# klasmodin/quflow

Measured on AMD Instinct MI355X. Metric: isospectral timesteps/sec at N=1024 (1 GPU) + ensemble steps/sec at 1/2/4/8 GPUs, higher is better.
Workload: dtype f64

## Files before the change

quflow_amd/csrc/api_context.hip:

```cpp
#include <cmath>
#include <cstdarg>
#include <cstdio>
#include <cstdlib>
#include <cstring>
#include <limits>
#include <chrono>

#include "qf_api.h"

static thread_local char g_err[512] = "";

void qf_set_error(const char *fmt, ...)
{
    va_list ap;
    va_start(ap, fmt);
    vsnprintf(g_err, sizeof(g_err), fmt, ap);
    va_end(ap);
}

extern "C" {

int qf_version(void) { return QF_VERSION; }

int qf_device_info(int device, char *buf, int n)
// ... 92 lines not shown
        if (g[0] == 'i' && strstr(g, "x6")) ctx->oz_digits = 6;
        if (g[0] == 'i' && strstr(g, "x65")) ctx->oz_digits2 = 5;
        if (g[0] == 'i' && strchr(g, 'h')) ctx->gemm_i8_hybrid = true;
        if (g[0] == 'i' && strchr(g, 'f') && !ctx->gemm_i8_hybrid) ctx->gemm_i8_first = true;
        if (g[0] == 'a') {
            ctx->gemm_i8_allowed = true;
            ctx->oz_digits = 6;
            ctx->oz_digits2 = 5;
            ctx->gemm_i8_min_n = 1024;
        }
    }
    if (const char *g = getenv("QUFLOW_HIP_GEMM2")) ctx->gemm_tri_allowed = !(g[0] == 'f');
    if (const char *g = getenv("QUFLOW_HIP_FUSED")) ctx->fused_allowed = !(g[0] == '0');
    if (const char *g = getenv("QUFLOW_HIP_I8_MIN_N")) ctx->gemm_i8_min_n = atoi(g);
    if (const char *g = getenv("QUFLOW_HIP_TRI_MIN_N")) ctx->gemm_tri_min_n = atoi(g);
    if (const char *g = getenv("QUFLOW_HIP_DEFER")) ctx->defer_allowed = !(g[0] == '0');
    if (getenv("QUFLOW_HIP_DEBUG"))
        if (const char *g = getenv("QUFLOW_HIP_DEBUG_DROP_FLAG")) ctx->debug_drop = atoi(g);
    if (const char *g = getenv("QUFLOW_HIP_FACTOR_CACHE_MB")) ctx->factor_budget_bytes = (size_t)(atoi(g) > 0 ? atoi(g) : 1) << 20;
    const size_t NN = (size_t)N * N;
    const size_t mbytes = NN * sizeof(cplx);
    int rc = QF_OK;
    auto fail = [&](int code) {
        qf_ctx_destroy(ctx);
        return code;
    };
#define QF_CREATE_HIP(call)                                                                   \
    do {                                                                                      \
        hipError_t _e = (call);                                                               \
        if (_e != hipSuccess) {                                                               \
// ... 288 lines not shown
```

quflow_amd/csrc/api_isomp.hip:

```cpp
#include <cmath>
#include <cstdarg>
#include <cstdio>
#include <cstdlib>
#include <cstring>
#include <limits>
#include <chrono>
#include <type_traits>
#include <utility>

#include "qf_api.h"

namespace {

#ifndef QF_RUN_AHEAD
#define QF_RUN_AHEAD 3
#endif

template <class S> constexpr bool is_c64 = std::is_same<S, qf_c64>::value;

template <class S> S *ws(qf_ctx *ctx)
{
    if constexpr (is_c64<S>) return ctx->c64;
    else return ctx;
}
// ... 61 lines not shown
        int so = 2, sd = 1;
        {
            const int cus = ctx->num_cus > 0 ? ctx->num_cus : 256;
            if (nt * (nt - 1) + 2 * nt <= cus) sd = 2;
            else if (nt * (nt - 1) + nt > cus) so = 1;
        }
        ctx->tri32_split = so;
        ctx->tri32_split_diag = sd;
    }
    return QF_OK;
}

int select_second_product(qf_ctx *ctx)
{
    ctx->gemm_tri = false;
    ctx->gemm_tri32 = false;
    ctx->gemm_i8 = false;
    const bool want_tri = ctx->gemm_tri_allowed && ctx->sk_partial && ctx->N >= ctx->gemm_tri_min_n;
    const size_t nt32 = (size_t)(ctx->N + 31) / 32;
    const bool tri32_fits = nt32 * (nt32 + 1) / 2 * 4 * 32 * 32 * sizeof(cplx) <= (size_t)0x7fffffff;
    const bool want_tri32 = ctx->gemm_tri_allowed && !want_tri && ctx->N >= 64 && tri32_fits;
    const bool want_i8 = ctx->gemm_i8_allowed && ctx->N % 64 == 0 && ctx->N >= ctx->gemm_i8_min_n && ctx->N <= 4096;
    if (!want_tri && !want_i8 && !want_tri32) return QF_OK;
    QF_TRY(check_skew(ctx, ctx));
    const bool skew = ctx->w_skew_known;
    ctx->gemm_tri = want_tri && skew;
    ctx->gemm_i8 = want_i8 && skew;
    ctx->gemm_tri32 = want_tri32 && skew && (!ctx->gemm_i8 || ctx->gemm_i8_first);
    if (ctx->gemm_tri32) QF_TRY(tri32_alloc(ctx));
    return QF_OK;
}

int select_second_product_c64(qf_ctx *ctx)
{
    qf_c64 *f = ctx->c64;
    f->tri = false;
    if (f->tri_allowed && ctx->gemm_tri_allowed && (qf_c64_tile(ctx) == 32 || ctx->N % 64 == 0) && ctx->N >= 64) {
        QF_TRY(check_skew(ctx, f));
        if (f->w_skew_known) {
            QF_TRY(qf_c64_tri_alloc(ctx));
            f->tri = true;
// ... 723 lines not shown
        QF_TRY(qf_launch_mirror_lower(ctx, f->dW[1]));
        QF_TRY(qf_launch_sum_rowpart(ctx, f->rowpart, (N + qf_c64_tile(ctx) - 1) / qf_c64_tile(ctx), ctx->rowsum));
    } else {
        QF_TRY(qf_launch_cgemm(ctx, f->PW, f->Phalf, nullptr, &ep));
        QF_TRY(qf_launch_sum_rowpart(ctx, f->rowpart, f->rowpart_tiles, ctx->rowsum));
    }
    QF_HIP(hipMemcpyAsync(dW_new_host, f->dW[1], bytes, hipMemcpyDeviceToHost, ctx->stream));
    QF_HIP(hipMemcpyAsync(Whalf_new_host, f->Whalf, bytes, hipMemcpyDeviceToHost, ctx->stream));
    QF_HIP(hipMemcpyAsync(rowsum_host, ctx->rowsum, (size_t)N * sizeof(double), hipMemcpyDeviceToHost, ctx->stream));
    QF_HIP(hipStreamSynchronize(ctx->stream));
    return QF_OK;
}

}

int qf_rowpart_slots(const qf_ctx *ctx) { return ctx->gemm_tri ? ctx->N / 64 : ctx->gemm_tri32 ? (ctx->N + 31) / 32 : ctx->rowpart_tiles; }

int qf_enqueue_diagnostics(qf_ctx *ctx)
{
    QF_TRY(qf_launch_solve(ctx, ctx->poisson, ctx->W, ctx->stage, 1.0, 1));
    QF_TRY(qf_launch_inner2(ctx, ctx->W, ctx->stage, ctx->scalars + 2));
    QF_HIP(hipMemcpyAsync(ctx->host_scalars, ctx->scalars + 2, 2 * sizeof(double), hipMemcpyDeviceToHost, ctx->stream));
    return QF_OK;
}

int qf_isomp_multi(qf_ctx **ctxs, int k, double dt, int steps, double tol, int minit, int maxit, qf_isomp_stats *stats_out)
{
    return isomp_multi<qf_ctx>(ctxs, k, dt, steps, tol, minit, maxit, stats_out);
}

int qf_c64_isomp_multi(qf_ctx **ctxs, int k, double dt, int steps, double tol, int minit, int maxit, qf_isomp_stats *stats_out)
// ... 30 lines not shown
    return QF_OK;
}


int qf_fixedpoint_products(qf_ctx *ctx, const void *Phalf_host, const void *Whalf_host, const void *W_host,
                           const void *dW_old_host, int variant, void *dW_new_host, void *Whalf_new_host,
                           double *rowsum_host)
{
    QF_TRY(check_ctx(ctx));
    if (!Phalf_host || !Whalf_host || !W_host || !dW_old_host || !dW_new_host || !Whalf_new_host || !rowsum_host) {
        qf_set_error("qf_fixedpoint_products: null buffer");
        return QF_ERR_INVALID;
    }
    const int variant_arg = variant;
    variant &= 15;
    if (variant == 1 && !ctx->sk_partial) {
        qf_set_error("qf_fixedpoint_products: the upper-triangle product needs N %% 64 == 0 (N=%d)", ctx->N);
        return QF_ERR_INVALID;
    }
    if (variant == 2) {
        if (ctx->N < 64) {
            qf_set_error("qf_fixedpoint_products: the 32x32 upper-triangle product needs N >= 64 (N=%d)", ctx->N);
            return QF_ERR_INVALID;
        }
        QF_TRY(tri32_alloc(ctx));
    }
    const int N = ctx->N;
    const size_t bytes = (size_t)N * N * sizeof(cplx);
    QF_HIP(hipMemcpyAsync(ctx->Phalf, Phalf_host, bytes, hipMemcpyHostToDevice, ctx->stream));
    QF_HIP(hipMemcpyAsync(ctx->Whalf, Whalf_host, bytes, hipMemcpyHostToDevice, ctx->stream));
    QF_HIP(hipMemcpyAsync(ctx->stage, W_host, bytes, hipMemcpyHostToDevice, ctx->stream));
    QF_HIP(hipMemcpyAsync(ctx->dW[0], dW_old_host, bytes, hipMemcpyHostToDevice, ctx->stream));
    QF_TRY(qf_launch_zgemm(ctx, ctx->Phalf, ctx->Whalf, ctx->PW, nullptr));
    qf_epilogue ep = epilogue_of(ctx, false);
    ep.W = ctx->stage;
    const bool saved = ctx->gemm_tri, saved32 = ctx->gemm_tri32;
    const int s_min = ctx->sk_min_units, s_epi = ctx->sk_epi_units, s_so = ctx->tri32_split, s_sd = ctx->tri32_split_diag;
    ctx->gemm_tri = (variant == 1);
    ctx->gemm_tri32 = (variant == 2);
    if (variant == 1) {
        if ((variant_arg >> 8) & 0xff) ctx->sk_min_units = (variant_arg >> 8) & 0xff;
        if ((variant_arg >> 16) & 0xff) ctx->sk_epi_units = ((variant_arg >> 16) & 0xff) - 64;
    } else if (variant == 2) {
        const int so = (variant_arg >> 8) & 15, sd = (variant_arg >> 12) & 15;
        if (so == 1 || so == 2 || so == 4) ctx->tri32_split = so;
        if (sd == 1 || sd == 2 || sd == 4) ctx->tri32_split_diag = sd;
    }
    int rc = qf_launch_zgemm(ctx, ctx->PW, ctx->Phalf, nullptr, &ep);
    ctx->gemm_tri = saved;
    ctx->gemm_tri32 = saved32;
    ctx->sk_min_units = s_min;
    ctx->sk_epi_units = s_epi;
    ctx->tri32_split = s_so;
    ctx->tri32_split_diag = s_sd;
    QF_TRY(rc);
    QF_TRY(qf_launch_sum_rowpart(ctx, ctx->rowpart, variant == 1 ? ctx->N / 64 : variant == 2 ? (ctx->N + 31) / 32 : ctx->rowpart_tiles, ctx->rowsum));
    QF_HIP(hipMemcpyAsync(dW_new_host, ctx->dW[1], bytes, hipMemcpyDeviceToHost, ctx->stream));
    QF_HIP(hipMemcpyAsync(Whalf_new_host, ctx->Whalf, bytes, hipMemcpyDeviceToHost, ctx->stream));
    QF_HIP(hipMemcpyAsync(rowsum_host, ctx->rowsum, (size_t)N * sizeof(double), hipMemcpyDeviceToHost, ctx->stream));
    QF_HIP(hipStreamSynchronize(ctx->stream));
    return QF_OK;
}


int qf_oz_alloc(qf_ctx *ctx)
{
    for (int q = 0; q < 4; ++q) {
        if (!ctx->oz_planes[q]) QF_HIP(hipMalloc((void **)&ctx->oz_planes[q], qf_oz_operand_bytes(ctx->N, ctx->oz_digits)));
        if (!ctx->oz_scale[q])
            QF_HIP(hipMalloc((void **)&ctx->oz_scale[q], qf_oz_record_bytes(ctx->N, ctx->oz_digits)));
    }
// ... 39 lines not shown
```

quflow_amd/csrc/api_steppers.hip:

```cpp
#include <cmath>
#include <cstdarg>
#include <cstdio>
#include <cstdlib>
#include <cstring>
#include <limits>
#include <chrono>

#include "qf_api.h"

extern "C" {

int qf_erk(qf_ctx *ctx, int method, double dt, int steps, int skewh)
{
    QF_TRY(check_ctx(ctx));
    if (method < QF_ERK_EULER || method > QF_ERK_RK4) {
        qf_set_error("qf_erk: unknown method %d", method);
        return QF_ERR_INVALID;
    }
    if (steps < 0) {
        qf_set_error("qf_erk: steps must be >= 0");
        return QF_ERR_INVALID;
    }
    const double inv_hb = 1.0 / qf_hbar(ctx->N);
    ctx->w_skew_known = false;
// ... 396 lines not shown
        QF_HIP(hipMemcpyAsync(S[j].X, (const char *)states_host + (size_t)j * mbytes, mbytes, hipMemcpyHostToDevice, ctx->stream));
        QF_HIP(hipMemsetAsync(S[j].dX[0], 0, mbytes, ctx->stream));
        QF_HIP(hipMemcpyAsync(S[j].Xhalf, S[j].X, mbytes, hipMemcpyDeviceToDevice, ctx->stream));
    }
    cplx *Bhalf = magnetic ? ctx->multi[5 * k] : nullptr;
    cplx *BT = magnetic ? ctx->multi[5 * k + 1] : nullptr;
    cplx *BTP = magnetic ? ctx->multi[5 * k + 2] : nullptr;

    bool tri = ctx->gemm_tri_allowed && ctx->sk_partial && N >= ctx->gemm_tri_min_n;
    for (int j = 0; j < k && tri; ++j) {
        QF_TRY(qf_launch_skew_defect(ctx, S[j].X, ctx->scalars + 4));
        QF_HIP(hipMemcpyAsync(ctx->host_scalars, ctx->scalars + 4, 2 * sizeof(double), hipMemcpyDeviceToHost, ctx->stream));
        QF_HIP(hipStreamSynchronize(ctx->stream));
        tri = (ctx->host_scalars[0] == 0.0);
    }
    const bool tri_saved = ctx->gemm_tri, tri32_saved = ctx->gemm_tri32;
    ctx->gemm_tri = tri;
    ctx->gemm_tri32 = false;
    auto restore = [&](int rc) { ctx->gemm_tri = tri_saved; ctx->gemm_tri32 = tri32_saved; return rc; };
#define QF_TRY_R(call)                  \
    do {                                \
        int _r = (call);                \
        if (_r != QF_OK) return restore(_r); \
    } while (0)

    if (tol < 0) {
        double nrm = 0.0;
        QF_TRY_R(qf_launch_norm_inf(ctx, S[0].X, ctx->scalars));
        QF_TRY_R(read_scalar(ctx, ctx->scalars, &nrm));
        tol = (std::sqrt(std::numeric_limits<double>::epsilon()) * dt / hb) * nrm;
    }

    long long total_iterations = 0, number_of_maxit = 0;
    double resnorm = 0.0;
// ... 56 lines not shown
                }
            }
        }
        if (!broke) number_of_maxit += 1;
        for (int j = 0; j < k; ++j)
            QF_TRY_R(qf_launch_update(ctx, S[j].PXc, S[j].X, S[j].dX[S[j].cur], S[j].dX[S[j].cur], S[j].Xhalf, nullptr,
                                      reinitialize));
        if (magnetic)
            QF_TRY_R(qf_launch_magnetic_update(ctx, BT, S[0].X, reinitialize ? nullptr : S[0].dX[S[0].cur], S[0].Xhalf));
    }
    for (int j = 0; j < k; ++j)
        QF_HIP(hipMemcpyAsync((char *)states_host + (size_t)j * mbytes, S[j].X, mbytes, hipMemcpyDeviceToHost, ctx->stream));
    QF_HIP(hipStreamSynchronize(ctx->stream));
#undef QF_TRY_R
    ctx->gemm_tri = tri_saved;
    ctx->gemm_tri32 = tri32_saved;
    if (stats_out) {
        stats_out->total_iterations = total_iterations;
        stats_out->number_of_maxit = number_of_maxit;
        stats_out->tol_used = tol;
        stats_out->last_resnorm = resnorm;
    }
    return QF_OK;
}


}
```

quflow_amd/csrc/qf_api.h:

```cpp
#pragma once

#include "qf_internal.h"

#include <sched.h>

namespace {
int drain_events(qf_ctx *ctx);

struct prof_scope {
    qf_ctx *ctx;
    qf_event_pair ev;
    bool active;
    prof_scope(qf_ctx *c, int id) : ctx(c), active(((c->profile_mask >> id) & 1) != 0)
    {
        ctx->plan_role = id;
        if (!active) return;
        if ((ctx->prof_seen[id]++ % ctx->profile_stride) != 0) {
            active = false;
            return;
        }
        if (ctx->events_free.empty()) {
            if (hipEventCreate(&ev.start) != hipSuccess || hipEventCreate(&ev.stop) != hipSuccess) {
                active = false;
                return;
// ... 48 lines not shown
}

int read_scalar(qf_ctx *ctx, const double *dev, double *out)
{
    QF_HIP(hipMemcpyAsync(ctx->host_scalars, dev, sizeof(double), hipMemcpyDeviceToHost, ctx->stream));
    QF_HIP(hipStreamSynchronize(ctx->stream));
    *out = ctx->host_scalars[0];
    return QF_OK;
}

}

extern "C" {
int qf_need_c64(qf_ctx *ctx);
int qf_oz_alloc(qf_ctx *ctx);
int qf_rowpart_slots(const qf_ctx *ctx);
int qf_enqueue_diagnostics(qf_ctx *ctx);
}
```

quflow_amd/csrc/qf_internal.h:

```cpp
#pragma once

#include <hip/hip_runtime.h>

#include <atomic>
#include <cstdarg>
#include <cstdio>
#include <map>
#include <mutex>
#include <string>
#include <vector>

#include "../../include/quflow_hip.h"

typedef double2 cplx;

hipError_t qf_guard_malloc(void **p, size_t bytes);
hipError_t qf_guard_free(void *p);
#define hipMalloc(p, n) qf_guard_malloc((void **)(p), (n))
#define hipFree(p) qf_guard_free((void *)(p))

void qf_set_error(const char *fmt, ...);
struct qf_ctx;
inline void qf_plan_note(qf_ctx *ctx, unsigned long long key, const char *fmt, ...) __attribute__((format(printf, 3, 4)));

// ... 262 lines not shown
    qf_sht sht;
    qf_eigh_ws eigh;

    double *rowpart = nullptr;
    int rowpart_tiles = 0;
    double *rowsum = nullptr;
    double *scalars = nullptr;
    double *host_scalars = nullptr;
    qf_dev_state *state = nullptr;
    qf_host_record *host_rec = nullptr;
    bool diag_at_exit = false, diag_valid = false;
    unsigned *ticket = nullptr;
    int pred_iters = 3;
    bool gemm_tri_allowed = true;
    bool gemm_tri = false;
    int gemm_tri_min_n = 960;
    bool gemm_tri32 = false;
    int tri32_split = 2, tri32_split_diag = 1;
    cplx *t32_partial = nullptr;
    unsigned *t32_arrive = nullptr;
    bool defer_allowed = true;
    bool defer = false;
    int num_cus = 0;
    cplx *sk_partial = nullptr;
    unsigned *sk_flags = nullptr;
    int sk_slots = 0;
    unsigned sk_epoch = 0;
    int sk_epi_units = 0;
    int sk_epi_units_fused = 2;
    int sk_min_units = 8;
// ... 174 lines not shown
```

quflow_amd/csrc/zgemm.hip:

```cpp
#include "qf_internal.h"
#include "qf_step_end.h"

#include <cstring>

typedef double v4d __attribute__((ext_vector_type(4)));

#ifdef QF_STAMP
__device__ unsigned long long *qf_stamp_buf = nullptr;
#define QF_STAMP_SLOTS 80
#ifdef QF_STAMP_LIGHT
#define QF_STAMP_AT(slot_)
#define QF_STAMP_PH(kt_, ph_)
__device__ unsigned long long *qf_phase_buf = nullptr;
#else
#define QF_STAMP_AT(slot_)                                                              \
    if (qf_stamp_buf && lane == 0 && (slot_) < QF_STAMP_SLOTS)                          \
        qf_stamp_buf[((size_t)blockIdx.x * (T / 64) + wave) * QF_STAMP_SLOTS + (slot_)] = __builtin_amdgcn_s_memtime();
__device__ unsigned long long *qf_phase_buf = nullptr;
#define QF_STAMP_PH(kt_, ph_)                                                           \
    if (qf_phase_buf && tid == 0 && (kt_) >= 20 && (kt_) < 28)                          \
        qf_phase_buf[((size_t)blockIdx.x * 8 + ((kt_) - 20)) * 5 + (ph_)] = __builtin_amdgcn_s_memtime();
#endif
__device__ unsigned long long *qf_tri_buf = nullptr;
#define QF_TRI_STAMP(seg_, k_)                                                          \
// ... 973 lines not shown
        t = n_t;
        k0 = n_k0;
        KT = n_KT;
        tm = n_tm;
        tn = n_tn;
        asm volatile("s_waitcnt lgkmcnt(0)\n\ts_barrier" ::: "memory");
    }
    if (run_finale)
        qf_fused_step_end(N, nt, ep.rowpart, sk.ticket, sk.state_rw, sk.rec, guard.iter, tid, reinterpret_cast<double *>(smem_raw));
#undef QF_TRI_NEXT
#undef QF_TRI_KOF
#undef QF_TRI_HAS_PIECE
#undef QF_TRI_START_LOADS
}

template <bool EXACT>
__global__ __launch_bounds__(256) void k_zgemm_tri32(int N, int nt, const cplx *__restrict__ A, const cplx *__restrict__ B,
                                                      qf_epilogue ep, qf_guard guard, qf_tri32 sx)
{
    if (!qf_guard_iter(guard)) return;
    constexpr int BM = 32, BN = 32, WM = 2, WN = 2;
    constexpr bool EPI = true, FAST = false;
    using SM = tile_smem<BM, BN, false>;
    constexpr int T = WM * WN * 64;
    constexpr int WTM = BM / WM, WTN = BN / WN;
    constexpr int MT = WTM / 16, NT = WTN / 16;
    static_assert(MT == 1 && NT == 1, "one MFMA tile per wave");
    constexpr int A_STRIDE = SM::A_STRIDE, B_STRIDE = SM::B_STRIDE;
    constexpr int A_PER = (BM * BK) / T, B_PER = (BN * BK) / T;
    constexpr int A_ROWS_PER = T / BK, B_ROWS_PER = T / BN;
// ... 363 lines not shown
}

int qf_gemm_tiles_n(int N)
{
    gemm_cfg c = pick_gemm(N);
    return (N + c.BN - 1) / c.BN;
}

int qf_launch_zgemm_tri(qf_ctx *ctx, const cplx *A, const cplx *B, const qf_epilogue *ep, qf_guard guard)
{
    const int N = ctx->N;
    if (!ep || N % 64 != 0 || !ctx->sk_partial || ctx->num_cus < 1) {
        qf_set_error("qf_launch_zgemm_tri: not available for this context (N=%d)", N);
        return QF_ERR_STATE;
    }
    static qf_smem_attr attr;
    QF_TRY(qf_smem_attr_set(attr, (const void *)k_zgemm_tri, ctx->device, TRI_SMEM_BYTES));
    const int nt = N / 64;
    int E = ep->fused ? ctx->sk_epi_units_fused : ctx->sk_epi_units;
    if (E < -8) E = -8;
    const long long units = (long long)nt * (nt + 1) / 2 * (N / BK + E);
    if (units > 0x7fffffffLL) {
        qf_set_error("qf_launch_zgemm_tri: N=%d is too large for the stream-K partition", N);
        return QF_ERR_INVALID;
    }
    long long grid_ll = units / (ctx->sk_min_units > 0 ? ctx->sk_min_units : 1);
    if (grid_ll > ctx->num_cus) grid_ll = ctx->num_cus;
    if (grid_ll < 1) grid_ll = 1;
    const int grid = (int)grid_ll;
    qf_streamk sk;
    const int slots = ctx->sk_slots > 0 ? ctx->sk_slots : ctx->num_cus;
    sk.slots = slots;
    sk.partial = ctx->sk_partial;
    sk.flags = ctx->sk_flags;
    sk.epoch = ++ctx->sk_epoch;
    sk.fault = &ctx->host_rec->fault;
    sk.ticket = ctx->sk_flags + slots;
    sk.n_tiles = nt * (nt + 1) / 2;
    sk.state_rw = ctx->state;
    sk.rec = ctx->host_rec;
    if (ctx->debug_drop == 1 || (ctx->debug_drop == 2 && ep->fused)) {
        sk.debug_drop = ctx->debug_drop;
        sk.spin_limit = 1u << 14;
        ctx->debug_drop = 0;
    }
    qf_plan_note(ctx, 0x2000000ull | (unsigned long long)(grid << 8 | (E & 0x3f) << 1 | (ep->fused ? 1 : 0)),
                 "{\"kernel\": \"k_zgemm_tri\", \"arithmetic\": \"fp64 3M, v_mfma_f64_16x16x4_f64\", \"tile\": [64, 64], \"tiles\": %d, "
                 "\"tile_share\": %.6f, \"workgroups\": %d, \"threads\": 256, \"partition\": \"stream-K over (tile, K-tile) units, "
                 "contiguous ranges, epilogue weight E = %d K-tiles\", \"step_end\": \"%s\"}",
                 sk.n_tiles, (double)sk.n_tiles / ((double)nt * nt), grid, E, ep->fused ? "fused (last finisher decides)" : "two-kernel");
    hipLaunchKernelGGL(k_zgemm_tri, dim3(grid), dim3(256), TRI_SMEM_BYTES, ctx->stream, N, nt, (int)units, E, A, B, *ep, guard, sk);
    QF_HIP(hipGetLastError());
    return QF_OK;
}

int qf_launch_zgemm_tri32(qf_ctx *ctx, const cplx *A, const cplx *B, const qf_epilogue *ep, qf_guard guard)
{
    const int N = ctx->N;
    if (!ep || N < 64 || !ctx->t32_partial || !ctx->t32_arrive) {
        qf_set_error("qf_launch_zgemm_tri32: not available for this context (N=%d)", N);
        return QF_ERR_STATE;
    }
    const int nt = (N + 31) / 32;
    qf_tri32 sx;
    sx.partial = ctx->t32_partial;
    sx.arrive = ctx->t32_arrive;
// ... 36 lines not shown
```

Before: 2699.

## Add half-tile stream-K units for triangular ZGEMM when tiles underfill CUs

Adds a k_zgemm_tri_half kernel that splits each 64x64 upper-triangle tile into two 64x32 column halves, doubling the number of stream-K work units. It is selected automatically when the triangular tile count is below the CU count but at least half of it, and N is at most 1024. The goal is better CU load balance and less idle hardware in the second fixed-point product. In exchange, tiles are smaller with lower data reuse, the epilogue and mirroring logic gets more complex, and there are more rowpart slots to sum.

New measurement: 2692. Within noise of the previous version (-0.3%).

```diff
diff --git a/quflow_amd/csrc/api_context.hip b/quflow_amd/csrc/api_context.hip
--- a/quflow_amd/csrc/api_context.hip
+++ b/quflow_amd/csrc/api_context.hip
@@ -130,6 +130,7 @@
     if (const char *g = getenv("QUFLOW_HIP_FUSED")) ctx->fused_allowed = !(g[0] == '0');
     if (const char *g = getenv("QUFLOW_HIP_I8_MIN_N")) ctx->gemm_i8_min_n = atoi(g);
     if (const char *g = getenv("QUFLOW_HIP_TRI_MIN_N")) ctx->gemm_tri_min_n = atoi(g);
+    if (const char *g = getenv("QUFLOW_HIP_TRI_UNIT")) ctx->tri_unit_mode = (g[0] == 't') ? 1 : (g[0] == 'h') ? 2 : 0;
     if (const char *g = getenv("QUFLOW_HIP_DEFER")) ctx->defer_allowed = !(g[0] == '0');
     if (getenv("QUFLOW_HIP_DEBUG"))
         if (const char *g = getenv("QUFLOW_HIP_DEBUG_DROP_FLAG")) ctx->debug_drop = atoi(g);
diff --git a/quflow_amd/csrc/api_isomp.hip b/quflow_amd/csrc/api_isomp.hip
--- a/quflow_amd/csrc/api_isomp.hip
+++ b/quflow_amd/csrc/api_isomp.hip
@@ -99,6 +99,7 @@
 int select_second_product(qf_ctx *ctx)
 {
     ctx->gemm_tri = false;
+    ctx->gemm_tri_half = false;
     ctx->gemm_tri32 = false;
     ctx->gemm_i8 = false;
     const bool want_tri = ctx->gemm_tri_allowed && ctx->sk_partial && ctx->N >= ctx->gemm_tri_min_n;
@@ -110,6 +111,7 @@
     QF_TRY(check_skew(ctx, ctx));
     const bool skew = ctx->w_skew_known;
     ctx->gemm_tri = want_tri && skew;
+    ctx->gemm_tri_half = ctx->gemm_tri && qf_tri_half_units(ctx);
     ctx->gemm_i8 = want_i8 && skew;
     ctx->gemm_tri32 = want_tri32 && skew && (!ctx->gemm_i8 || ctx->gemm_i8_first);
     if (ctx->gemm_tri32) QF_TRY(tri32_alloc(ctx));
@@ -863,7 +865,15 @@
 
 }
 
-int qf_rowpart_slots(const qf_ctx *ctx) { return ctx->gemm_tri ? ctx->N / 64 : ctx->gemm_tri32 ? (ctx->N + 31) / 32 : ctx->rowpart_tiles; }
+bool qf_tri_half_units(const qf_ctx *ctx)
+{
+    if (ctx->N % 64 != 0 || !ctx->sk_partial || ctx->tri_unit_mode == 1) return false;
+    if (ctx->tri_unit_mode == 2) return true;
+    const int nt = ctx->N / 64, n_tiles = nt * (nt + 1) / 2;
+    return n_tiles < ctx->num_cus && ctx->num_cus <= 2 * n_tiles && ctx->N <= ctx->tri_half_max_n;
+}
+
+int qf_rowpart_slots(const qf_ctx *ctx) { return ctx->gemm_tri ? (ctx->gemm_tri_half ? ctx->N / 32 : ctx->N / 64) : ctx->gemm_tri32 ? (ctx->N + 31) / 32 : ctx->rowpart_tiles; }
 
 int qf_enqueue_diagnostics(qf_ctx *ctx)
 {
@@ -924,7 +934,7 @@
     }
     const int variant_arg = variant;
     variant &= 15;
-    if (variant == 1 && !ctx->sk_partial) {
+    if ((variant == 1 || variant == 3) && !ctx->sk_partial) {
         qf_set_error("qf_fixedpoint_products: the upper-triangle product needs N %% 64 == 0 (N=%d)", ctx->N);
         return QF_ERR_INVALID;
     }
@@ -944,11 +954,12 @@
     QF_TRY(qf_launch_zgemm(ctx, ctx->Phalf, ctx->Whalf, ctx->PW, nullptr));
     qf_epilogue ep = epilogue_of(ctx, false);
     ep.W = ctx->stage;
-    const bool saved = ctx->gemm_tri, saved32 = ctx->gemm_tri32;
+    const bool saved = ctx->gemm_tri, saved32 = ctx->gemm_tri32, saved_half = ctx->gemm_tri_half;
     const int s_min = ctx->sk_min_units, s_epi = ctx->sk_epi_units, s_so = ctx->tri32_split, s_sd = ctx->tri32_split_diag;
-    ctx->gemm_tri = (variant == 1);
+    ctx->gemm_tri = (variant == 1 || variant == 3);
+    ctx->gemm_tri_half = (variant == 3);
     ctx->gemm_tri32 = (variant == 2);
-    if (variant == 1) {
+    if (variant == 1 || variant == 3) {
         if ((variant_arg >> 8) & 0xff) ctx->sk_min_units = (variant_arg >> 8) & 0xff;
         if ((variant_arg >> 16) & 0xff) ctx->sk_epi_units = ((variant_arg >> 16) & 0xff) - 64;
     } else if (variant == 2) {
@@ -958,13 +969,14 @@
     }
     int rc = qf_launch_zgemm(ctx, ctx->PW, ctx->Phalf, nullptr, &ep);
     ctx->gemm_tri = saved;
+    ctx->gemm_tri_half = saved_half;
     ctx->gemm_tri32 = saved32;
     ctx->sk_min_units = s_min;
     ctx->sk_epi_units = s_epi;
     ctx->tri32_split = s_so;
     ctx->tri32_split_diag = s_sd;
     QF_TRY(rc);
-    QF_TRY(qf_launch_sum_rowpart(ctx, ctx->rowpart, variant == 1 ? ctx->N / 64 : variant == 2 ? (ctx->N + 31) / 32 : ctx->rowpart_tiles, ctx->rowsum));
+    QF_TRY(qf_launch_sum_rowpart(ctx, ctx->rowpart, variant == 1 ? ctx->N / 64 : (variant == 2 || variant == 3) ? (ctx->N + 31) / 32 : ctx->rowpart_tiles, ctx->rowsum));
     QF_HIP(hipMemcpyAsync(dW_new_host, ctx->dW[1], bytes, hipMemcpyDeviceToHost, ctx->stream));
     QF_HIP(hipMemcpyAsync(Whalf_new_host, ctx->Whalf, bytes, hipMemcpyDeviceToHost, ctx->stream));
     QF_HIP(hipMemcpyAsync(rowsum_host, ctx->rowsum, (size_t)N * sizeof(double), hipMemcpyDeviceToHost, ctx->stream));
diff --git a/quflow_amd/csrc/api_steppers.hip b/quflow_amd/csrc/api_steppers.hip
--- a/quflow_amd/csrc/api_steppers.hip
+++ b/quflow_amd/csrc/api_steppers.hip
@@ -434,10 +434,11 @@
         QF_HIP(hipStreamSynchronize(ctx->stream));
         tri = (ctx->host_scalars[0] == 0.0);
     }
-    const bool tri_saved = ctx->gemm_tri, tri32_saved = ctx->gemm_tri32;
+    const bool tri_saved = ctx->gemm_tri, tri32_saved = ctx->gemm_tri32, half_saved = ctx->gemm_tri_half;
     ctx->gemm_tri = tri;
+    ctx->gemm_tri_half = tri && qf_tri_half_units(ctx);
     ctx->gemm_tri32 = false;
-    auto restore = [&](int rc) { ctx->gemm_tri = tri_saved; ctx->gemm_tri32 = tri32_saved; return rc; };
+    auto restore = [&](int rc) { ctx->gemm_tri = tri_saved; ctx->gemm_tri_half = half_saved; ctx->gemm_tri32 = tri32_saved; return rc; };
 #define QF_TRY_R(call)                  \
     do {                                \
         int _r = (call);                \
@@ -524,6 +525,7 @@
     QF_HIP(hipStreamSynchronize(ctx->stream));
 #undef QF_TRY_R
     ctx->gemm_tri = tri_saved;
+    ctx->gemm_tri_half = half_saved;
     ctx->gemm_tri32 = tri32_saved;
     if (stats_out) {
         stats_out->total_iterations = total_iterations;
diff --git a/quflow_amd/csrc/qf_api.h b/quflow_amd/csrc/qf_api.h
--- a/quflow_amd/csrc/qf_api.h
+++ b/quflow_amd/csrc/qf_api.h
@@ -86,6 +86,7 @@
 extern "C" {
 int qf_need_c64(qf_ctx *ctx);
 int qf_oz_alloc(qf_ctx *ctx);
+bool qf_tri_half_units(const qf_ctx *ctx);
 int qf_rowpart_slots(const qf_ctx *ctx);
 int qf_enqueue_diagnostics(qf_ctx *ctx);
 }
diff --git a/quflow_amd/csrc/qf_internal.h b/quflow_amd/csrc/qf_internal.h
--- a/quflow_amd/csrc/qf_internal.h
+++ b/quflow_amd/csrc/qf_internal.h
@@ -300,6 +300,9 @@
     int pred_iters = 3;
     bool gemm_tri_allowed = true;
     bool gemm_tri = false;
+    bool gemm_tri_half = false;
+    int tri_unit_mode = 0;
+    int tri_half_max_n = 1024;
     int gemm_tri_min_n = 960;
     bool gemm_tri32 = false;
     int tri32_split = 2, tri32_split_diag = 1;
diff --git a/quflow_amd/csrc/zgemm.hip b/quflow_amd/csrc/zgemm.hip
--- a/quflow_amd/csrc/zgemm.hip
+++ b/quflow_amd/csrc/zgemm.hip
@@ -1011,6 +1011,529 @@
 #undef QF_TRI_START_LOADS
 }
 
+constexpr size_t TRIH_EPI_BYTES = 3 * 64 * 33 * sizeof(cplx) + (64 + 4 * 32) * sizeof(double) + 64;
+constexpr size_t TRIH_SMEM_BYTES = tile_smem<64, 32, true>::main_bytes > TRIH_EPI_BYTES ? tile_smem<64, 32, true>::main_bytes : TRIH_EPI_BYTES;
+
+__global__ __launch_bounds__(256) void k_zgemm_tri_half(int N, int nt, int U, int E, const cplx *__restrict__ A,
+                                                         const cplx *__restrict__ B, qf_epilogue ep, qf_guard guard,
+                                                         qf_streamk sk)
+{
+    constexpr int BM = 64, BN = 32;
+    constexpr bool FAST = true;
+    using SM = tile_smem<BM, BN, true>;
+    constexpr int T = 256;
+    constexpr int WTM = 32;
+    constexpr int MT = 2, NT = 2;
+    constexpr int A_STRIDE = SM::A_STRIDE, B_STRIDE = SM::B_STRIDE;
+    constexpr int A_PER = (BM * BK) / T, B_PER = (BN * BK) / T;
+    constexpr int A3_STRIDE = SM::A3_STRIDE, B3_STRIDE = SM::B3_STRIDE;
+    constexpr int TS = BN + 1;
+    constexpr int TT_BYTES = BM * TS * (int)sizeof(cplx);
+    static_assert((size_t)3 * TT_BYTES + (BM + 4 * BN) * sizeof(double) + 16 <= TRIH_SMEM_BYTES, "epilogue scratch exceeds the LDS request");
+    static_assert(TRIH_SMEM_BYTES >= SM::main_bytes && TRIH_SMEM_BYTES <= TRI_SMEM_BYTES, "LDS request");
+    static_assert(A_PER == 4 && B_PER == 2, "staging maps below");
+    typedef unsigned v4u __attribute__((ext_vector_type(4)));
+    constexpr int SG_MFMA = 0x008, SG_VMEM_RD = 0x020, SG_DS_WR = 0x200;
+
+    extern __shared__ __attribute__((aligned(16))) unsigned char smem_raw[];
+
+    const int tid = threadIdx.x;
+    const int lane = tid & 63, wave = tid >> 6;
+    const int wm = wave >> 1, kh = wave & 1;
+    const int r16_c = lane & 15, q4_c = lane >> 4;
+    const int G = gridDim.x;
+    const int c = xcd_remap(blockIdx.x, G);
+    const int KTN = N / BK;
+    const int S = KTN + E;
+    const int uq = U / G, ur = U % G;
+#define QF_H_CUT(c_) ((int)(c_) * uq + (int)(((unsigned)(c_) * (unsigned)ur) / (unsigned)G))
+    int u = QF_H_CUT(c);
+    const int u_end = QF_H_CUT(c + 1);
+    const cplx zero = make_double2(0.0, 0.0);
+
+    const unsigned char *lds_fa[2] = {
+        smem_raw + (size_t)((kh * 8 + q4_c) * A_STRIDE + wm * WTM + (r16_c ^ q4_c)) * sizeof(cplx),
+        smem_raw + (size_t)((kh * 8 + q4_c) * A_STRIDE + wm * WTM + (r16_c ^ q4_c ^ 4)) * sizeof(cplx)};
+    const unsigned char *lds_fb = smem_raw + SM::B_OFFSET + (size_t)((kh * 8 + q4_c) * B_STRIDE + r16_c) * sizeof(cplx);
+    unsigned char *lds_sa = smem_raw + (size_t)((tid % BK) * A_STRIDE + ((tid / BK) ^ (tid % BK & 7))) * sizeof(cplx);
+    const unsigned char *lds_fa3[2] = {
+        smem_raw + SM::A3_OFFSET + (size_t)((kh * 8 + q4_c) * A3_STRIDE + wm * WTM + 2 * (r16_c ^ q4_c)) * sizeof(double),
+        smem_raw + SM::A3_OFFSET + (size_t)((kh * 8 + q4_c) * A3_STRIDE + wm * WTM + 2 * (r16_c ^ q4_c ^ 4)) * sizeof(double)};
+    const unsigned char *lds_fb3 = smem_raw + SM::B3_OFFSET + (size_t)((kh * 8 + q4_c) * B3_STRIDE + 2 * r16_c) * sizeof(double);
+    unsigned char *lds_sa3 = smem_raw + SM::A3_OFFSET + (size_t)((tid % BK) * A3_STRIDE + 2 * ((tid / BK) ^ (tid % BK & 7))) * sizeof(double);
+    unsigned char *lds_sb = smem_raw + SM::B_OFFSET + (size_t)((tid / 16) * B_STRIDE + (tid % 16)) * sizeof(cplx);
+    unsigned char *lds_sb3 = smem_raw + SM::B3_OFFSET + (size_t)((tid / 16) * B3_STRIDE + 2 * (tid % 16)) * sizeof(double);
+    const __amdgpu_buffer_rsrc_t rsrcA = __builtin_amdgcn_make_buffer_rsrc(const_cast<cplx *>(A), 0, (int)((size_t)N * N * sizeof(cplx)), 0x00020000);
+    const __amdgpu_buffer_rsrc_t rsrcB = __builtin_amdgcn_make_buffer_rsrc(const_cast<cplx *>(B), 0, (int)((size_t)N * N * sizeof(cplx)), 0x00020000);
+    const unsigned fa_voff = (unsigned)(((size_t)(tid / BK) * N + (tid % BK)) * sizeof(cplx));
+    const unsigned fb_voff = (unsigned)(((size_t)(tid / 16) * N + (tid % 16)) * sizeof(cplx));
+    const unsigned f_rows16 = (unsigned)((size_t)16 * N * sizeof(cplx));
+    const __amdgpu_buffer_rsrc_t rsrcP = __builtin_amdgcn_make_buffer_rsrc(sk.partial, 0, (int)((size_t)sk.slots * (64 * 64) * sizeof(cplx)), 0x00020000);
+    const unsigned p_voff = (unsigned)(tid * sizeof(cplx));
+
+    cplx e_c[NT][4], e_t[NT][4], e_w[NT][4], e_old[NT][4];
+    v4d accR[MT][NT], accI[MT][NT], accS[MT][NT];
+    cplx ra[2][A_PER], rb[2][B_PER];
+    cplx fa[2][MT], fb[2][NT];
+    double fas[2][MT], fbs[2][NT];
+#pragma unroll
+    for (int r = 0; r < A_PER; ++r) ra[1][r] = zero;
+#pragma unroll
+    for (int r = 0; r < B_PER; ++r) rb[1][r] = zero;
+
+#define QF_H_KOF(p_) ((p_) <= 0 ? 0 : ((p_) <= E + 1 ? 1 : ((p_) - E > KTN ? KTN : (int)((p_) - E))))
+#define QF_H_NEXT(u_, found_, t_, k0_, KT_, tm_, tn_, hf_)                             \
+    {                                                                                  \
+        found_ = false;                                                                \
+        while (!(found_) && (u_) < u_end) {                                            \
+            t_ = (int)((u_) / S);                                                      \
+            const int pa_ = (u_) - (t_) * S;                                           \
+            int pb_ = u_end - (t_) * S;                                                \
+            if (pb_ > S) pb_ = S;                                                      \
+            const int klo_ = QF_H_KOF(pa_), khi_ = QF_H_KOF(pb_);                      \
+            u_ = (t_) * S + pb_;                                                       \
+            if (klo_ < khi_) {                                                         \
+                found_ = true;                                                         \
+                k0_ = klo_;                                                            \
+                KT_ = khi_ - klo_;                                                     \
+                int rem_ = (t_) >> 1;                                                  \
+                hf_ = (t_) & 1;                                                        \
+                tm_ = 0;                                                               \
+                while (rem_ >= nt - (tm_)) { rem_ -= nt - (tm_); ++(tm_); }            \
+                tn_ = (tm_) + rem_;                                                    \
+            }                                                                          \
+        }                                                                              \
+    }
+#define QF_H_LOAD(kt_, SET_)                                                           \
+    {                                                                                  \
+        const unsigned kc_ = (unsigned)((kt_) >= KT ? KT - 1 : (kt_));                 \
+        const unsigned sa_ = fa_soff0 + kc_ * (unsigned)(BK * sizeof(cplx));           \
+        const unsigned sb_ = fb_soff0 + kc_ * f_rows16;                                \
+        _Pragma("unroll") for (int r = 0; r < A_PER; ++r)                              \
+        {                                                                              \
+            const v4u t_ = __builtin_amdgcn_raw_buffer_load_b128(rsrcA, fa_voff, sa_ + r * f_rows16, 0); \
+            ra[SET_][r] = *reinterpret_cast<const cplx *>(&t_);                        \
+        }                                                                              \
+        _Pragma("unroll") for (int r = 0; r < B_PER; ++r)                              \
+        {                                                                              \
+            const v4u t_ = __builtin_amdgcn_raw_buffer_load_b128(rsrcB, fb_voff + r * 256u, sb_, 0); \
+            rb[SET_][r] = *reinterpret_cast<const cplx *>(&t_);                        \
+        }                                                                              \
+    }
+#define QF_H_STORE(BUF_, SET_)                                                         \
+    {                                                                                  \
+        _Pragma("unroll") for (int r = 0; r < A_PER; ++r)                              \
+            *reinterpret_cast<cplx *>(lds_sa + (BUF_) * SM::A_BUF_BYTES + r * 16 * (int)sizeof(cplx)) = ra[SET_][r]; \
+        _Pragma("unroll") for (int h = 0; h < 2; ++h)                                  \
+            *reinterpret_cast<double2 *>(lds_sa3 + (BUF_) * SM::A3_BUF_BYTES + h * 32 * (int)sizeof(double)) =             \
+                make_double2(QF_SUM3M(ra[SET_][2 * h]), QF_SUM3M(ra[SET_][2 * h + 1]));       \
+        _Pragma("unroll") for (int r = 0; r < B_PER; ++r)                              \
+            *reinterpret_cast<cplx *>(lds_sb + (BUF_) * SM::B_BUF_BYTES + r * 16 * (int)sizeof(cplx)) = rb[SET_][r]; \
+        *reinterpret_cast<double2 *>(lds_sb3 + (BUF_) * SM::B3_BUF_BYTES) = make_double2(QF_SUM3M(rb[SET_][0]), QF_SUM3M(rb[SET_][1])); \
+    }
+#define QF_H_START_LOADS(k0_, KT_, tm_, tn_, hf_)                                      \
+    {                                                                                  \
+        const int kt_of_segment_ = (KT_);                                              \
+        fa_soff0 = (unsigned)(((size_t)(tm_) * BM * N + (size_t)(k0_) * BK) * sizeof(cplx)); \
+        fb_soff0 = (unsigned)(((size_t)(k0_) * BK * N + (size_t)(tn_) * 64 + (size_t)(hf_) * BN) * sizeof(cplx)); \
+        {                                                                              \
+            const int KT = kt_of_segment_;        \
+            QF_H_LOAD(0, 0)                                                            \
+            if (KT > 1) { QF_H_LOAD(1, 1) }                                            \
+        }                                                                              \
+    }
+#define QF_H_FETCH(dst_, src_, TRANSPOSED_)                                            \
+    {                                                                                  \
+        _Pragma("unroll") for (int ni = 0; ni < NT; ++ni)                              \
+            _Pragma("unroll") for (int reg = 0; reg < 4; ++reg)                        \
+        {                                                                              \
+            const int gi = i0 + wave * 16 + q4 + 4 * reg;                              \
+            const int gj = j0 + ni * 16 + r16;                                         \
+            dst_[ni][reg] = (TRANSPOSED_) ? (src_)[(size_t)gj * N + gi] : (src_)[(size_t)gi * N + gj]; \
+        }                                                                              \
+    }
+#define QF_H_COMM                                                                      \
+    {                                                                                  \
+        _Pragma("unroll") for (int ni = 0; ni < NT; ++ni)                              \
+            _Pragma("unroll") for (int reg = 0; reg < 4; ++reg)                        \
+        {                                                                              \
+            e_c[ni][reg].x = e_c[ni][reg].x - e_t[ni][reg].x;                          \
+            e_c[ni][reg].y = e_c[ni][reg].y + e_t[ni][reg].y;                          \
+        }                                                                              \
+    }
+#define QF_H_KTILE(kt_, BUF_, PREF_)                                                   \
+    {                                                                                  \
+        QF_READ_FRAGS(1, BUF_, 1)                                                      \
+        __builtin_amdgcn_sched_barrier(0);                                             \
+        if (!QF_ABL_NOSTORE) { QF_H_STORE((BUF_) ^ 1, (BUF_) ^ 1) }                    \
+        if ((PREF_) == 1) QF_H_FETCH(e_c, ep.PW, false)                                \
+        if ((PREF_) == 2) QF_H_FETCH(e_t, ep.PW, true)                                 \
+        if ((PREF_) == 3) QF_H_COMM                                                    \
+        QF_MFMA(0)                                                                     \
+        _Pragma("unroll") for (int g = 0; g < A_PER + 2 + B_PER + 1; ++g)              \
+        {                                                                              \
+            __builtin_amdgcn_sched_group_barrier(SG_MFMA, 1, 0);                       \
+            __builtin_amdgcn_sched_group_barrier(SG_DS_WR, 1, 0);                      \
+        }                                                                              \
+        __builtin_amdgcn_sched_barrier(0);                                             \
+         \
+        if (QF_ABL_NOBARRIER) asm volatile("s_waitcnt lgkmcnt(0)" ::: "memory");      \
+        else asm volatile("s_waitcnt lgkmcnt(0)\n\ts_barrier" ::: "memory");           \
+        __builtin_amdgcn_sched_barrier(0);                                             \
+        QF_READ_FRAGS(0, (BUF_) ^ 1, 0)                                                \
+        __builtin_amdgcn_sched_barrier(0);                                             \
+        if (!QF_ABL_NOGLOAD) { QF_H_LOAD((kt_) + 3, (BUF_) ^ 1) }                      \
+        QF_MFMA(1)                                                                     \
+        _Pragma("unroll") for (int g = 0; g < A_PER + B_PER; ++g)                      \
+        {                                                                              \
+            __builtin_amdgcn_sched_group_barrier(SG_MFMA, 1, 0);                       \
+            __builtin_amdgcn_sched_group_barrier(SG_VMEM_RD, 1, 0);                    \
+        }                                                                              \
+        __builtin_amdgcn_sched_barrier(0);                                             \
+        __builtin_amdgcn_s_waitcnt(0xC07F);                                            \
+        __builtin_amdgcn_sched_barrier(0);                                             \
+    }
+
+    int seg = 0;
+    (void)seg;
+    bool run_finale = false;
+    int t = 0, k0 = 0, KT = 0, tm = 0, tn = 0, hf = 0;
+    unsigned fa_soff0 = 0, fb_soff0 = 0;
+    bool have = false;
+    QF_H_NEXT(u, have, t, k0, KT, tm, tn, hf)
+    if (have) QF_H_START_LOADS(k0, KT, tm, tn, hf)
+    if (!qf_guard_iter(guard)) have = false;
+    const int parity = guard.state ? guard.state->dw_parity : 0;
+    const cplx *__restrict__ ep_dW_old = ep.dW[parity];
+    cplx *__restrict__ ep_dW_new = ep.dW[parity ^ 1];
+    const int wpar = (ep.fused && guard.state) ? guard.state->w_parity : 0;
+    const cplx *__restrict__ ep_W = ep.fused ? ep.Wpair[wpar] : ep.W;
+    cplx *__restrict__ ep_Wnext = ep.fused ? ep.Wpair[wpar ^ 1] : nullptr;
+    const bool below_maxit = ep.fused && sk.state_rw && (guard.iter + 1 < sk.state_rw->maxit);
+    const bool open_for_sure = below_maxit && (guard.iter + 1 < sk.state_rw->minit);
+    const bool open_if_large = below_maxit && guard.iter == 0;
+    const double tol_now = (ep.fused && sk.state_rw) ? sk.state_rw->tol : 0.0;
+
+    while (have) {
+        const int i0 = tm * BM, j0 = tn * 64 + hf * BN;
+        const bool head = (k0 == 0);
+        int r16 = r16_c, q4 = q4_c, lane_v = lane;
+        asm volatile("" : "+v"(r16), "+v"(q4), "+v"(lane_v));
+#pragma unroll
+        for (int a = 0; a < MT; ++a)
+#pragma unroll
+            for (int b = 0; b < NT; ++b) {
+                accR[a][b] = (v4d){0.0, 0.0, 0.0, 0.0};
+                accI[a][b] = (v4d){0.0, 0.0, 0.0, 0.0};
+                accS[a][b] = (v4d){0.0, 0.0, 0.0, 0.0};
+            }
+
+        QF_TRI_STAMP(seg, 0)
+        QF_TRI_NOTE(seg, 4, k0)
+        QF_TRI_NOTE(seg, 5, KT)
+        QF_H_STORE(0, 0)
+        __syncthreads();
+        if (KT > 2) { QF_H_LOAD(2, 0) }
+        QF_READ_FRAGS(0, 0, 0)
+        __builtin_amdgcn_s_waitcnt(0xC07F);
+
+        QF_TRI_STAMP(seg, 6)
+        int kt = 0;
+        const bool spread = head && KT >= 10;
+        if (spread) {
+            QF_H_KTILE(0, 0, 0)
+            QF_H_KTILE(1, 1, 1)
+            QF_H_KTILE(2, 0, 2)
+            QF_H_KTILE(3, 1, 0)
+            QF_H_KTILE(4, 0, 3)
+            QF_H_KTILE(5, 1, 0)
+            kt = 6;
+        }
+        for (; kt + 1 < KT; kt += 2) {
+            QF_H_KTILE(kt, 0, 0)
+            QF_H_KTILE(kt + 1, 1, 0)
+        }
+        if (kt < KT) { QF_H_KTILE(kt, 0, 0) }
+        QF_TRI_STAMP(seg, 1)
+
+        int n_t = 0, n_k0 = 0, n_KT = 0, n_tm = 0, n_tn = 0, n_hf = 0;
+        bool have_next = false;
+        QF_H_NEXT(u, have_next, n_t, n_k0, n_KT, n_tm, n_tn, n_hf)
+
+        if (head) {
+            if (!spread) {
+                QF_H_FETCH(e_c, ep.PW, false)
+                QF_H_FETCH(e_t, ep.PW, true)
+            }
+            QF_H_FETCH(e_w, ep_W, false)
+            QF_H_FETCH(e_old, ep_dW_old, false)
+        }
+        double gre[NT][4], gim[NT][4];
+        cplx pv[NT * 4];
+        bool have_piece = false;
+#pragma unroll
+        for (int q = 0; q < NT * 4; ++q) {
+            gre[q / 4][q % 4] = gim[q / 4][q % 4] = 0.0;
+            pv[q] = zero;
+        }
+        if (head && KT < KTN) {
+            const int tile_org = t * S, tile_end = tile_org + S;
+            const int c_first = c + 1;
+            int c_last = c;
+            while (c_last + 1 < G && QF_H_CUT(c_last + 1) < tile_end) ++c_last;
+#define QF_H_HAS_PIECE(c2_)                                                            \
+    (QF_H_KOF(QF_H_CUT(c2_) - tile_org) < QF_H_KOF((QF_H_CUT((c2_) + 1) < tile_end ? QF_H_CUT((c2_) + 1) : tile_end) - tile_org))
+            for (int c2 = c_last; c2 >= c_first; --c2) {
+                const int slot2 = c2;
+                if (!QF_H_HAS_PIECE(c2)) continue;
+                if (tid == 0) {
+                    unsigned spins = 0;
+                    while (__hip_atomic_load(sk.flags + slot2, __ATOMIC_RELAXED, __HIP_MEMORY_SCOPE_AGENT) != sk.epoch) {
+                        __builtin_amdgcn_s_sleep(QF_POLL_SLEEP);
+                        if (++spins > sk.spin_limit) {
+                            *sk.fault = 1;
+                            break;
+                        }
+                    }
+                }
+                asm volatile("s_barrier" ::: "memory");
+#pragma unroll
+                for (int q = 0; q < NT * 4; ++q) {
+                    gre[q / 4][q % 4] += pv[q].x;
+                    gim[q / 4][q % 4] += pv[q].y;
+                }
+                const unsigned soff = (unsigned)((size_t)slot2 * (64 * 64) * sizeof(cplx));
+#pragma unroll
+                for (int q = 0; q < NT * 4; ++q) {
+                    const v4u raw = __builtin_amdgcn_raw_buffer_load_b128(rsrcP, p_voff + (unsigned)(q * T * sizeof(cplx)), soff, QF_SK_AUX_LD);
+                    pv[q] = *reinterpret_cast<const cplx *>(&raw);
+                }
+                have_piece = true;
+            }
+        }
+        double tre[NT][4], tim[NT][4];
+        {
+            cplx *Pk = reinterpret_cast<cplx *>(smem_raw);
+            asm volatile("s_waitcnt lgkmcnt(0)\n\ts_barrier" ::: "memory");
+#pragma unroll
+            for (int mi = 0; mi < MT; ++mi)
+#pragma unroll
+                for (int ni = 0; ni < NT; ++ni)
+#pragma unroll
+                    for (int reg = 0; reg < 4; ++reg)
+                        Pk[(kh * BM + wm * WTM + mi * 16 + q4 + 4 * reg) * TS + ni * 16 + r16] =
+                            make_double2(accR[mi][ni][reg] - accI[mi][ni][reg], (accS[mi][ni][reg] - accR[mi][ni][reg]) - accI[mi][ni][reg]);
+            asm volatile("s_waitcnt lgkmcnt(0)\n\ts_barrier" ::: "memory");
+#pragma unroll
+            for (int ni = 0; ni < NT; ++ni)
+#pragma unroll
+                for (int reg = 0; reg < 4; ++reg) {
+                    const int e = (wave * 16 + q4 + 4 * reg) * TS + ni * 16 + r16;
+                    const cplx p0 = Pk[e], p1 = Pk[BM * TS + e];
+                    tre[ni][reg] = p0.x + p1.x;
+                    tim[ni][reg] = p0.y + p1.y;
+                }
+            asm volatile("s_waitcnt lgkmcnt(0)\n\ts_barrier" ::: "memory");
+        }
+
+        if (!head) {
+            const int park_slot = c;
+#pragma unroll
+            for (int ni = 0; ni < NT; ++ni)
+#pragma unroll
+                for (int reg = 0; reg < 4; ++reg) {
+                    const cplx v = make_double2(tre[ni][reg], tim[ni][reg]);
+                    __builtin_amdgcn_raw_buffer_store_b128(*reinterpret_cast<const v4u *>(&v), rsrcP,
+                                                           p_voff + (unsigned)((ni * 4 + reg) * T * sizeof(cplx)),
+                                                           (unsigned)((size_t)park_slot * (64 * 64) * sizeof(cplx)), QF_SK_AUX_ST);
+                }
+            asm volatile("s_waitcnt vmcnt(0)" ::: "memory");
+            if (have_next) QF_H_START_LOADS(n_k0, n_KT, n_tm, n_tn, n_hf)
+            __syncthreads();
+            if (tid == 0 && !(sk.debug_drop & 1)) __hip_atomic_store(sk.flags + park_slot, sk.epoch, __ATOMIC_RELAXED, __HIP_MEMORY_SCOPE_AGENT);
+            QF_TRI_STAMP(seg, 2)
+        } else {
+            if (!spread) QF_H_COMM
+            if (have_piece) {
+#pragma unroll
+                for (int ni = 0; ni < NT; ++ni)
+#pragma unroll
+                    for (int reg = 0; reg < 4; ++reg) {
+                        tre[ni][reg] += gre[ni][reg] + pv[ni * 4 + reg].x;
+                        tim[ni][reg] += gim[ni][reg] + pv[ni * 4 + reg].y;
+                    }
+            }
+            QF_TRI_STAMP(seg, 2)
+            cplx *Th = reinterpret_cast<cplx *>(smem_raw);
+            cplx *Ts = reinterpret_cast<cplx *>(smem_raw + TT_BYTES);
+            cplx *Td = reinterpret_cast<cplx *>(smem_raw + 2 * TT_BYTES);
+            double *rs = reinterpret_cast<double *>(smem_raw + 3 * TT_BYTES);
+            double *cs = rs + BM;
+            unsigned *open_flag = reinterpret_cast<unsigned *>(cs + 4 * BN);
+            const bool offdiag = (tm != tn);
+            const int mirror_rows = offdiag ? BM : (hf ? 32 : 0);
+            const bool live = offdiag || hf || wave < 2;
+            const bool mirror_dW = !ep.fused || !offdiag;
+
+#pragma unroll
+            for (int ni = 0; ni < NT; ++ni)
+#pragma unroll
+                for (int reg = 0; reg < 4; ++reg) {
+                    tre[ni][reg] += e_c[ni][reg].x;
+                    tim[ni][reg] += e_c[ni][reg].y;
+                }
+            if (!offdiag) {
+#pragma unroll
+                for (int ni = 0; ni < NT; ++ni)
+#pragma unroll
+                    for (int reg = 0; reg < 4; ++reg)
+                        Td[(wave * 16 + q4 + 4 * reg) * TS + ni * 16 + r16] = make_double2(tre[ni][reg], tim[ni][reg]);
+                asm volatile("s_waitcnt lgkmcnt(0)\n\ts_barrier" ::: "memory");
+                if ((wave >> 1) == hf) {
+#pragma unroll
+                    for (int ni = 0; ni < NT; ++ni)
+#pragma unroll
+                        for (int reg = 0; reg < 4; ++reg) {
+                            const int rb_ = (wave & 1) * 16 + q4 + 4 * reg, cb_ = ni * 16 + r16;
+                            const cplx m = Td[(hf * 32 + cb_) * TS + rb_];
+                            if (rb_ > cb_) {
+                                tre[ni][reg] = -m.x;
+                                tim[ni][reg] = m.y;
+                            } else if (rb_ == cb_) {
+                                tre[ni][reg] = 0.0;
+                            }
+                        }
+                }
+            }
+
+            double csum[NT] = {0.0, 0.0};
+            if (tid == 0) *open_flag = 0u;
+#pragma unroll
+            for (int reg = 0; reg < 4; ++reg) {
+                const int li = wave * 16 + q4 + 4 * reg;
+                double rsum = 0.0;
+#pragma unroll
+                for (int ni = 0; ni < NT; ++ni) {
+                    const int lj = ni * 16 + r16;
+                    const size_t e = (size_t)(i0 + li) * N + (j0 + lj);
+                    const double dr = tre[ni][reg], di = tim[ni][reg];
+                    const cplx w = e_w[ni][reg];
+                    const cplx wh = make_double2(w.x + dr, w.y + di);
+                    if (live) {
+                        ep_dW_new[e] = make_double2(dr, di);
+                        ep.Whalf[e] = wh;
+                    }
+                    Th[li * TS + lj] = wh;
+                    if (offdiag && mirror_dW) Td[li * TS + lj] = make_double2(dr, di);
+                    const cplx o = e_old[ni][reg];
+                    const double er = o.x - dr, ei = o.y - di;
+                    const double a = qf_modulus(er, ei);
+                    rsum += a;
+                    csum[ni] += a;
+                }
+                rsum = qf_row16_sum(rsum);
+                if (r16 == 0) rs[li] = rsum;
+            }
+            if (mirror_rows) {
+#pragma unroll
+                for (int ni = 0; ni < NT; ++ni) {
+                    double s2 = csum[ni];
+                    s2 += __shfl_xor(s2, 16, 64);
+                    s2 += __shfl_xor(s2, 32, 64);
+                    if (q4 == 0) cs[wave * BN + ni * 16 + r16] = s2;
+                }
+            }
+            asm volatile("s_waitcnt lgkmcnt(0)\n\ts_barrier" ::: "memory");
+            if (tid < BM) {
+                const double s2 = rs[tid];
+                if (offdiag || hf || tid < 32) {
+                __hip_atomic_store(ep.rowpart + (size_t)(2 * tn + hf) * N + i0 + tid, s2, __ATOMIC_RELAXED, __HIP_MEMORY_SCOPE_AGENT);
+                if (open_if_large && s2 > tol_now) *open_flag = 1u;
+                }
+            } else if (tid < BM + (mirror_rows / 32) * BN) {
+                const int half = (tid - BM) / BN, lj = (tid - BM) % BN;
+                const double s2 = cs[(2 * half) * BN + lj] + cs[(2 * half + 1) * BN + lj];
+                __hip_atomic_store(ep.rowpart + (size_t)(2 * tm + half) * N + j0 + lj, s2, __ATOMIC_RELAXED, __HIP_MEMORY_SCOPE_AGENT);
+                if (open_if_large && s2 > tol_now) *open_flag = 1u;
+            }
+            unsigned ticket_old = 0u;
+            if (ep.fused) {
+                asm volatile("s_waitcnt vmcnt(0) lgkmcnt(0)\n\ts_barrier" ::: "memory");
+                if (tid == 0 && !((sk.debug_drop & 2) && t == 0))
+                    ticket_old = __hip_atomic_fetch_add(sk.ticket, 1u, __ATOMIC_RELAXED, __HIP_MEMORY_SCOPE_AGENT);
+            } else {
+                asm volatile("s_waitcnt lgkmcnt(0)\n\ts_barrier" ::: "memory");
+            }
+            QF_TRI_STAMP(seg, 7)
+            const bool speculate = ep.fused && !(open_for_sure || (open_if_large && *open_flag != 0u));
+            if (speculate) {
+#pragma unroll
+                for (int reg = 0; reg < 4; ++reg) {
+                    const int li = wave * 16 + q4 + 4 * reg;
+#pragma unroll
+                    for (int ni = 0; ni < NT; ++ni) {
+                        const int lj = ni * 16 + r16;
+                        const size_t e = (size_t)(i0 + li) * N + (j0 + lj);
+                        const cplx w = e_w[ni][reg];
+                        const cplx wc = make_double2(w.x + 2.0 * e_c[ni][reg].x, w.y + 2.0 * e_c[ni][reg].y);
+                        const cplx whs = make_double2(wc.x + tre[ni][reg], wc.y + tim[ni][reg]);
+                        ep_Wnext[e] = wc;
+                        if (live) ep.Whalf_step[e] = whs;
+                        Ts[li * TS + lj] = whs;
+                    }
+                }
+            }
+            asm volatile("s_waitcnt lgkmcnt(0)\n\ts_barrier" ::: "memory");
+            if (lane_v < mirror_rows) {
+#pragma unroll
+                for (int r = 0; r < 8; ++r) {
+                    const int jl = wave * 8 + r;
+                    const cplx wv = Th[lane_v * TS + jl];
+                    const size_t e2 = (size_t)(j0 + jl) * N + (i0 + lane_v);
+                    ep.Whalf[e2] = make_double2(-wv.x, wv.y);
+                    if (speculate) {
+                        const cplx ws = Ts[lane_v * TS + jl];
+                        ep.Whalf_step[e2] = make_double2(-ws.x, ws.y);
+                    }
+                    if (mirror_dW) {
+                        const cplx wd = Td[lane_v * TS + jl];
+                        ep_dW_new[e2] = make_double2(-wd.x, wd.y);
+                    }
+                }
+            }
+            if (have_next) QF_H_START_LOADS(n_k0, n_KT, n_tm, n_tn, n_hf)
+            if (ep.fused) {
+                unsigned *last_flag = reinterpret_cast<unsigned *>(rs);
+                if (tid == 0) *last_flag = (ticket_old == (unsigned)(sk.n_tiles - 1)) ? 1u : 0u;
+                asm volatile("s_waitcnt lgkmcnt(0)\n\ts_barrier" ::: "memory");
+                if (*last_flag != 0u) run_finale = true;
+            }
+        }
+        QF_TRI_STAMP(seg, 3)
+        ++seg;
+        have = have_next;
+        t = n_t;
+        k0 = n_k0;
+        KT = n_KT;
+        tm = n_tm;
+        tn = n_tn;
+        hf = n_hf;
+        asm volatile("s_waitcnt lgkmcnt(0)\n\ts_barrier" ::: "memory");
+    }
+    if (run_finale)
+        qf_fused_step_end(N, 2 * nt, ep.rowpart, sk.ticket, sk.state_rw, sk.rec, guard.iter, tid, reinterpret_cast<double *>(smem_raw));
+#undef QF_H_NEXT
+#undef QF_H_KOF
+#undef QF_H_HAS_PIECE
+#undef QF_H_CUT
+#undef QF_H_START_LOADS
+#undef QF_H_LOAD
+#undef QF_H_STORE
+#undef QF_H_FETCH
+#undef QF_H_COMM
+#undef QF_H_KTILE
+}
+
 template <bool EXACT>
 __global__ __launch_bounds__(256) void k_zgemm_tri32(int N, int nt, const cplx *__restrict__ A, const cplx *__restrict__ B,
                                                       qf_epilogue ep, qf_guard guard, qf_tri32 sx)
@@ -1404,12 +1927,14 @@
         qf_set_error("qf_launch_zgemm_tri: not available for this context (N=%d)", N);
         return QF_ERR_STATE;
     }
-    static qf_smem_attr attr;
-    QF_TRY(qf_smem_attr_set(attr, (const void *)k_zgemm_tri, ctx->device, TRI_SMEM_BYTES));
+    const bool half = ctx->gemm_tri_half;
+    static qf_smem_attr attr, attr_half;
+    if (half) QF_TRY(qf_smem_attr_set(attr_half, (const void *)k_zgemm_tri_half, ctx->device, TRIH_SMEM_BYTES));
+    else QF_TRY(qf_smem_attr_set(attr, (const void *)k_zgemm_tri, ctx->device, TRI_SMEM_BYTES));
     const int nt = N / 64;
     int E = ep->fused ? ctx->sk_epi_units_fused : ctx->sk_epi_units;
     if (E < -8) E = -8;
-    const long long units = (long long)nt * (nt + 1) / 2 * (N / BK + E);
+    const long long units = (long long)nt * (nt + 1) / 2 * (half ? 2 : 1) * (N / BK + E);
     if (units > 0x7fffffffLL) {
         qf_set_error("qf_launch_zgemm_tri: N=%d is too large for the stream-K partition", N);
         return QF_ERR_INVALID;
@@ -1426,7 +1951,8 @@
     sk.epoch = ++ctx->sk_epoch;
     sk.fault = &ctx->host_rec->fault;
     sk.ticket = ctx->sk_flags + slots;
-    sk.n_tiles = nt * (nt + 1) / 2;
+    const int n_tiles = nt * (nt + 1) / 2;
+    sk.n_tiles = half ? 2 * n_tiles : n_tiles;
     sk.state_rw = ctx->state;
     sk.rec = ctx->host_rec;
     if (ctx->debug_drop == 1 || (ctx->debug_drop == 2 && ep->fused)) {
@@ -1434,12 +1960,14 @@
         sk.spin_limit = 1u << 14;
         ctx->debug_drop = 0;
     }
-    qf_plan_note(ctx, 0x2000000ull | (unsigned long long)(grid << 8 | (E & 0x3f) << 1 | (ep->fused ? 1 : 0)),
-                 "{\"kernel\": \"k_zgemm_tri\", \"arithmetic\": \"fp64 3M, v_mfma_f64_16x16x4_f64\", \"tile\": [64, 64], \"tiles\": %d, "
-                 "\"tile_share\": %.6f, \"workgroups\": %d, \"threads\": 256, \"partition\": \"stream-K over (tile, K-tile) units, "
+    qf_plan_note(ctx, (half ? 0x2800000ull : 0x2000000ull) | (unsigned long long)(grid << 8 | (E & 0x3f) << 1 | (ep->fused ? 1 : 0)),
+                 "{\"kernel\": \"k_zgemm_tri\", \"arithmetic\": \"fp64 3M, v_mfma_f64_16x16x4_f64\", \"tile\": [64, %d], \"tiles\": %d, "
+                 "\"tile_share\": %.6f, \"workgroups\": %d, \"threads\": 256, \"partition\": \"stream-K over (%s, K-tile) units, "
                  "contiguous ranges, epilogue weight E = %d K-tiles\", \"step_end\": \"%s\"}",
-                 sk.n_tiles, (double)sk.n_tiles / ((double)nt * nt), grid, E, ep->fused ? "fused (last finisher decides)" : "two-kernel");
-    hipLaunchKernelGGL(k_zgemm_tri, dim3(grid), dim3(256), TRI_SMEM_BYTES, ctx->stream, N, nt, (int)units, E, A, B, *ep, guard, sk);
+                 half ? 32 : 64, n_tiles, (double)n_tiles / ((double)nt * nt), grid, half ? "half-tile units: 64 x 32 column half" : "tile",
+                 E, ep->fused ? "fused (last finisher decides)" : "two-kernel");
+    if (half) hipLaunchKernelGGL(k_zgemm_tri_half, dim3(grid), dim3(256), TRIH_SMEM_BYTES, ctx->stream, N, nt, (int)units, E, A, B, *ep, guard, sk);
+    else hipLaunchKernelGGL(k_zgemm_tri, dim3(grid), dim3(256), TRI_SMEM_BYTES, ctx->stream, N, nt, (int)units, E, A, B, *ep, guard, sk);
     QF_HIP(hipGetLastError());
     return QF_OK;
 }
```
